# kuwt/model_matching

Measured on AMD Instinct MI355X. Metric: candidate poses verified/sec, higher is better.
Workload: dtype f32; 1 GPU; Cm: synthetic 20000-pt scene vs 5000-pt model, 65536 candidate transforms per step per GPU, eps=5mm; scene_points=20000, model_points=5000

## Files before the change

model_matching_amd/csrc/lcp.hip:

```cpp
#include <stdlib.h>
#include <string.h>

#include <cstring>


#include <algorithm>
#include <utility>

#include "kdtree.h"
#include "prims.h"
#include "stocs_ctx.h"

namespace stocs {

struct LcpArgs {
    const float4* mpos;
    const float4* mnrm;
    const int32_t* mperm;
    int M;
    const int32_t* top;
    const uint4* cells;
    const uint4* flat;
    const float4* list;
    const float4* snrmw;
// ... 165 lines not shown
    __shared__ unsigned long long part[WPB];
    const int lane = threadIdx.x & 63;
    const int sub = lane & 7, grp = lane >> 3;
    const int w = threadIdx.x >> 6;
    const int cand = SPLIT ? lcp_candidate(a, n, 0, 1) : lcp_candidate(a, n, w, WPB);
    if (cand < 0) return;
    const int first = SPLIT ? 64 * w : 0, stride = SPLIT ? 64 * WPB : 64;
    const float4* __restrict__ snrmw = lcp_weights_of(a, cand);
    const float* T = T16 + (size_t)cand * 16;
    const float t0 = T[0], t1 = T[1], t2 = T[2], t4 = T[4], t5 = T[5], t6 = T[6], t8 = T[8], t9 = T[9], t10 = T[10],
                t12 = T[12], t13 = T[13], t14 = T[14];
    unsigned long long acc = 0ull;
    for (int base = first; base < a.M; base += stride) {
        const int i = base + lane;
        float qx = 0.f, qy = 0.f, qz = 0.f, qcd = 0.f;
        uint32_t off = 0, cnt = 0;
        if (i < a.M) {
            const float4 p = a.mpos[i];
            qx = ((t0 * p.x + t4 * p.y) + t8 * p.z) + t12;
            qy = ((t1 * p.x + t5 * p.y) + t9 * p.z) + t13;
            qz = ((t2 * p.x + t6 * p.y) + t10 * p.z) + t14;
            const float ux = (qx - a.ox) * a.inv_h, uy = (qy - a.oy) * a.inv_h, uz = (qz - a.oz) * a.inv_h;
            const float fx = floorf(ux), fy = floorf(uy), fz = floorf(uz);
            if (fx >= 0.0f && fy >= 0.0f && fz >= 0.0f && fx < (float)a.nx && fy < (float)a.ny && fz < (float)a.nz) {
                const int cx = (int)fx, cy = (int)fy, cz = (int)fz;
                const int brick = STOCS_ABLATE(a, 1) ? -1 : a.top[((cz >> 3) * a.nby + (cy >> 3)) * a.nbx + (cx >> 3)];
                if (brick >= 0) {
                    uint4 cw = make_uint4(0u, 0u, 0u, 0u);
                    if (!STOCS_ABLATE(a, 128)) cw = a.cells[(size_t)brick * 512 + (((cz & 7) << 6) | ((cy & 7) << 3) | (cx & 7))];
                    const int sb = ((int)((uz - fz) * 4.0f) << 4) | ((int)((uy - fy) * 4.0f) << 2) | (int)((ux - fx) * 4.0f);
                    const uint32_t mw = a.has_nearest ? 0xFFFFFFFFu : (sb < 32 ? cw.z : cw.w);
                    off = cw.x; cnt = ((mw >> (sb & 31)) & 1u) ? cw.y : 0u;
                    if (STOCS_ABLATE(a, 2)) cnt = cw.x == 0xFFFFFFF1u ? 1u : 0u;
                    const float ex = qx - (a.ox + ((float)cx + 0.5f) * a.h), ey = qy - (a.oy + ((float)cy + 0.5f) * a.h),
                                ez = qz - (a.oz + ((float)cz + 0.5f) * a.h);
                    qcd = sqrtf(ex * ex + (ey * ey + ez * ez));
                }
            }
        }
        const bool hit = cnt != 0;
        const unsigned long long mask = __ballot(hit);
        int best = -1;
        if (mask) {
            const int nh = __popcll(mask);
            if (hit) {
                const int rank = __popcll(mask & ((1ull << lane) - 1ull));
                hl[w][rank] = (uint32_t)lane;
                qt[w][lane] = make_float4(qx, qy, qz, __int_as_float((int)off));
                qn[w][lane] = cnt;
                qd[w][lane] = qcd;
            }
            __builtin_amdgcn_wave_barrier();
            for (int s = 0; s < nh; s += 8) {
                const int slot = s + grp;
                const bool gact = slot < nh;
                const uint32_t L = gact ? hl[w][slot] : 0u;
                const float4 qq = qt[w][L];
                const uint32_t c = gact ? qn[w][L] : 0u;
                const float4* lp = a.list + (uint32_t)__float_as_int(qq.w) + sub;
                float gd = a.sq_eps;
                int gi = -1;
                const float qcg = qd[w][L];
                const uint32_t chunk0 = (uint32_t)__float_as_int(qq.w) >> 3;
                uint32_t nchunks = (c + 7u) >> 3;
                float gb = a.sq_eps;
                if (STOCS_ABLATE(a, 4)) nchunks = min(nchunks, (uint32_t)UNR);
                for (uint32_t j = 0; __any(j < nchunks); j += UNR) {
                    if (j < nchunks && j > 0 && (STOCS_ABLATE(a, 256) ? 0.0f : a.chunk_r[chunk0 + j]) - qcg > sqrtf(gb) + a.bound_margin) nchunks = 0;
                    float4 e[UNR];
#pragma unroll
                    for (int u = 0; u < UNR; ++u) {
                        e[u] = make_float4(1e30f, 1e30f, 1e30f, __int_as_float(-1));
                        if (j + u < nchunks) e[u] = lp[(j + u) << 3];
                    }
#pragma unroll
                    for (int u = 0; u < UNR; ++u) {
                        const float dx = qq.x - e[u].x, dy = qq.y - e[u].y, dz = qq.z - e[u].z;
                        const float d = dx * dx + (dy * dy + dz * dz);
                        const int ei = __float_as_int(e[u].w);
                        if (d < gd || (d == gd && ei > gi)) { gd = d; gi = ei; }
                    }
                    gb = fminf(gd, dpp_f32<DPP_QUAD_XOR1>(gd));
                    gb = fminf(gb, dpp_f32<DPP_QUAD_XOR2>(gb));
                    gb = fminf(gb, dpp_f32<DPP_HALF_MIRROR>(gb));
                }
                float dm = fminf(gd, dpp_f32<DPP_QUAD_XOR1>(gd));
                dm = fminf(dm, dpp_f32<DPP_QUAD_XOR2>(dm));
                dm = fminf(dm, dpp_f32<DPP_HALF_MIRROR>(dm));
                int im = (gd == dm) ? gi : -1;
                im = max(im, dpp_i32<DPP_QUAD_XOR1>(im));
                im = max(im, dpp_i32<DPP_QUAD_XOR2>(im));
                im = max(im, dpp_i32<DPP_HALF_MIRROR>(im));
                if (gact && sub == 0) { rd[w][L] = dm; ri[w][L] = im; }
            }
            __builtin_amdgcn_wave_barrier();
            if (hit) best = ri[w][lane];
            __builtin_amdgcn_wave_barrier();
        }
        bool counted = false;
        if (best >= 0 && STOCS_ABLATE(a, 8)) lcp_add(acc, 0.5f);
        else if (best >= 0) {
            const float4 nm = a.mnrm[i];
            const float nx = t0 * nm.x + (t4 * nm.y + t8 * nm.z);
            const float ny = t1 * nm.x + (t5 * nm.y + t9 * nm.z);
            const float nz = t2 * nm.x + (t6 * nm.y + t10 * nm.z);
            const float4 sn = snrmw[best];
            const float d = sn.x * nx + (sn.y * ny + sn.z * nz);
            counted = (d >= a.dot_lo) && (d <= 1.0f);
            if (counted) lcp_add(acc, sn.w);
        }
        if (DETAIL && i < a.M) {
            const int orig = a.mperm[i];
            hit_out[(size_t)cand * a.M + orig] = best;
            cnt_out[(size_t)cand * a.M + orig] = counted ? 1 : 0;
        }
    }
    acc = lcp_wave_sum(acc);
    if (SPLIT) {
        if (lane == 0) part[w] = acc;
        __syncthreads();
        if (threadIdx.x == 0) {
            unsigned long long total = 0;
#pragma unroll
            for (int k = 0; k < WPB; ++k) total += part[k];
            lcp_store(a, out, cand, total);
        }
    } else if (lane == 0) lcp_store(a, out, cand, acc);
}

__device__ __forceinline__ float lcp_linear_norm_bound(float t0, float t1, float t2, float t4, float t5, float t6, float t8, float t9, float t10) {
    const float g00 = t0 * t0 + (t1 * t1 + t2 * t2), g11 = t4 * t4 + (t5 * t5 + t6 * t6), g22 = t8 * t8 + (t9 * t9 + t10 * t10);
    const float g01 = fabsf(t0 * t4 + (t1 * t5 + t2 * t6)), g02 = fabsf(t0 * t8 + (t1 * t9 + t2 * t10)), g12 = fabsf(t4 * t8 + (t5 * t9 + t6 * t10));
    const float rho = fmaxf(g00 + (g01 + g02), fmaxf(g11 + (g01 + g12), g22 + (g02 + g12)));
    return sqrtf(rho) * 1.00001f;
}
__device__ __forceinline__ bool lcp_patch_dead(const LcpArgs& a, const float4 sp, float sn, float t0, float t1, float t2, float t4, float t5, float t6,
                                               float t8, float t9, float t10, float t12, float t13, float t14) {
    const float cx = ((t0 * sp.x + t4 * sp.y) + t8 * sp.z) + t12;
    const float cy = ((t1 * sp.x + t5 * sp.y) + t9 * sp.z) + t13;
    const float cz = ((t2 * sp.x + t6 * sp.y) + t10 * sp.z) + t14;
    const float mag = fabsf(cx) + (fabsf(cy) + fabsf(cz));
    if (!(mag < 1.0e18f)) return false;
    const float need = (sn * sp.w + a.eps * 1.002f) + (4.0e-6f + 4.0e-6f * mag);
    const float ux = (cx - a.gox) * a.inv_g, uy = (cy - a.goy) * a.inv_g, uz = (cz - a.goz) * a.inv_g;
    const float fx = floorf(ux), fy = floorf(uy), fz = floorf(uz);
    if (fx >= 1.0f && fy >= 1.0f && fz >= 1.0f && fx < (float)(a.gnx - 1) && fy < (float)(a.gny - 1) && fz < (float)(a.gnz - 1)) {
        const float v = a.dist[((uint32_t)(int)fz * (uint32_t)a.gny + (uint32_t)(int)fy) * (uint32_t)a.gnx + (uint32_t)(int)fx];
        const float ex = cx - (a.gox + (fx + 0.5f) * a.g), ey = cy - (a.goy + (fy + 0.5f) * a.g), ez = cz - (a.goz + (fz + 0.5f) * a.g);
        return v - sqrtf(ex * ex + (ey * ey + ez * ez)) > need;
    }
    return a.cap > need;
}

constexpr bool lcp_queue_form_legal(bool detail, bool dense, bool split, bool flat, bool near, int cu) {
    return (cu == 16 || cu == 64) && (detail ? (!split && !flat && !(dense && near)) : (!dense || (split && !flat && !near)));
}

template <bool DETAIL, bool DENSE, bool SPLIT, bool FLAT, bool NEAR, int CU>
__global__ __launch_bounds__(64 * lcp_waves_per_block(DETAIL, SPLIT), 8) void lcp_coopq_kernel(LcpArgs a, const float* __restrict__ T16, float* __restrict__ out,
                                                        int n, int32_t* __restrict__ hit_out, uint8_t* __restrict__ cnt_out) {
    static_assert(lcp_queue_form_legal(DETAIL, DENSE, SPLIT, FLAT, NEAR, CU), "not one of the forms in the table above");
    constexpr int WPB = lcp_waves_per_block(DETAIL, SPLIT);
    constexpr bool IDX = !DENSE;
    constexpr bool EARLY = DENSE;
    constexpr int GL = 4, EPL = 8 / GL, NG = 64 / GL;
    constexpr int FIRST = DENSE ? 1 : 2, E0 = EPL * FIRST;
    constexpr bool NOSENT = !DENSE;
    constexpr int UNR = 1;
    constexpr int PIPE = 1;
    static_assert(!EARLY || (FIRST == 1 && !NOSENT), "early exit decides line by line");
    __shared__ float4 qt[WPB][128];
    __shared__ float qcd[EARLY ? WPB : 1][EARLY ? 128 : 1];
    __shared__ uint32_t qn[WPB][128];
    __shared__ uint32_t qs[WPB][128];
    __shared__ int ri[WPB][128];
    __shared__ uint8_t ord[WPB][64];
    __shared__ unsigned long long part[WPB];
    const int lane = threadIdx.x & 63;
    const int w = threadIdx.x >> 6;
    const int cand = SPLIT ? lcp_candidate(a, n, 0, 1) : lcp_candidate(a, n, w, WPB);
    if (cand < 0) return;
    const float4* __restrict__ snrmw = lcp_weights_of(a, cand);
    const float* T = T16 + (size_t)cand * 16;
    const float t0 = T[0], t1 = T[1], t2 = T[2], t4 = T[4], t5 = T[5], t6 = T[6], t8 = T[8], t9 = T[9], t10 = T[10],
                t12 = T[12], t13 = T[13], t14 = T[14];
    unsigned long long acc = 0ull;
    int head = 0, tail = 0;

    auto process = [&](int nq) {
        {
            uint32_t cls = 4;
            if (lane < nq) {
                const uint32_t nch = (qn[w][(head + lane) & 127] + 7u) >> 3;
                cls = nch <= (uint32_t)FIRST ? 1u : (nch <= (uint32_t)(FIRST + UNR) ? 2u : 3u);
            }
            const unsigned long long below = (1ull << lane) - 1ull;
            const unsigned long long m1 = __ballot(cls == 1u), m2 = __ballot(cls == 2u), m3 = __ballot(cls == 3u);
            const int n1 = __popcll(m1), n2 = __popcll(m2);
            const int pos = cls == 1u ? __popcll(m1 & below) : (cls == 2u ? n1 + __popcll(m2 & below) : n1 + n2 + __popcll(m3 & below));
            if (lane < nq) ord[w][pos] = (uint8_t)lane;
            __builtin_amdgcn_wave_barrier();
        }
        for (int s0 = 0; s0 < nq; s0 += NG * PIPE) {
            const int sub = lane & (GL - 1), grp = lane / GL;
            float4 e0[PIPE][E0];
            bool wide[PIPE];
            int idxs[PIPE];
            uint32_t cs[PIPE];
#pragma unroll
            for (int u = 0; u < PIPE; ++u) {
                const int slot = s0 + NG * u + grp;
                const bool gact = slot < nq;
                idxs[u] = (head + (int)ord[w][gact ? slot : 0]) & 127;
                cs[u] = gact ? qn[w][idxs[u]] : 0u;
                wide[u] = true;
                if (!NOSENT) {
#pragma unroll
                    for (int e = 0; e < E0; ++e) e0[u][e] = make_float4(1e30f, 1e30f, 1e30f, __int_as_float(-1));
                }
                if (STOCS_ABLATE(a, 4)) {
                    if (cs[u]) { const float4 qq0 = qt[w][idxs[u]]; e0[u][0] = make_float4(qq0.x, qq0.y, qq0.z, __int_as_float(0)); }
                    cs[u] = cs[u] ? 1u : 0u;
                }
                else if (NOSENT) {
                    const float4* l0 = a.list + (cs[u] ? (uint32_t)__float_as_int(qt[w][idxs[u]].w) : 0u) + sub;
                    const uint32_t last = cs[u] ? ((cs[u] - 1u) & ~7u) : 0u;
#pragma unroll
                    for (int e = 0; e < EPL; ++e) e0[u][e] = l0[GL * e];
                    wide[u] = FIRST > 1 && __any(cs[u] > 8u);
                    if (wide[u]) {
#pragma unroll
                        for (int e = EPL; e < E0; ++e) e0[u][e] = l0[min((uint32_t)(8 * (e / EPL)), last) + GL * (e % EPL)];
                    }
                }
                else if (cs[u]) {
                    const float4* l0 = a.list + (uint32_t)__float_as_int(qt[w][idxs[u]].w) + sub;
#pragma unroll
                    for (int e = 0; e < E0; ++e) e0[u][e] = l0[GL * e];
                }
            }
#pragma unroll
            for (int u = 0; u < PIPE; ++u) {
                const float4 qq = qt[w][idxs[u]];
                const uint32_t c = cs[u];
                const float4* lp = a.list + (uint32_t)__float_as_int(qq.w) + sub;
                const uint32_t last_line = c ? ((c - 1u) & ~7u) : 0u;
                float gd = a.sq_eps;
                int gi = -1;
#pragma unroll
                for (int e = 0; e < EPL; ++e) {
                    const float dx = qq.x - e0[u][e].x, dy = qq.y - e0[u][e].y, dz = qq.z - e0[u][e].z;
                    const float d = dx * dx + (dy * dy + dz * dz);
                    take_if_better<IDX>(d, __float_as_int(e0[u][e].w), gd, gi);
                }
                if (FIRST > 1 && wide[u]) {
#pragma unroll
                    for (int e = EPL; e < E0; ++e) {
                        const float dx = qq.x - e0[u][e].x, dy = qq.y - e0[u][e].y, dz = qq.z - e0[u][e].z;
                        const float d = dx * dx + (dy * dy + dz * dz);
                        take_if_better<IDX>(d, __float_as_int(e0[u][e].w), gd, gi);
                    }
                }
                if (EARLY) {
                    const float qcg = qcd[w][idxs[u]];
                    const uint32_t chunk0 = (uint32_t)__float_as_int(qq.w) >> 3;
                    uint32_t cc = c;
                    for (uint32_t k = 8; __any(k < cc); k += 8 * UNR) {
                        if (k < cc && a.chunk_r[chunk0 + (k >> 3)] - qcg > sqrtf(group_min_nonneg<GL>(gd)) + a.bound_margin) cc = 0;
                        float4 e[EPL];
                        if (k < cc) {
#pragma unroll
                            for (int x = 0; x < EPL; ++x) e[x] = lp[k + GL * x];
                        } else {
#pragma unroll
                            for (int x = 0; x < EPL; ++x) e[x] = make_float4(1e30f, 1e30f, 1e30f, __int_as_float(-1));
                        }
#pragma unroll
                        for (int x = 0; x < EPL; ++x) {
                            const float dx = qq.x - e[x].x, dy = qq.y - e[x].y, dz = qq.z - e[x].z;
                            const float d = dx * dx + (dy * dy + dz * dz);
                            take_if_better<IDX>(d, __float_as_int(e[x].w), gd, gi);
                        }
                    }
                } else {
                    for (uint32_t k = 8 * FIRST; __any(k < c); k += 8 * UNR) {
                        const uint32_t kk = min(k, last_line);
                        float4 e[EPL];
#pragma unroll
                        for (int x = 0; x < EPL; ++x) e[x] = lp[kk + GL * x];
#pragma unroll
                        for (int x = 0; x < EPL; ++x) {
                            const float dx = qq.x - e[x].x, dy = qq.y - e[x].y, dz = qq.z - e[x].z;
                            const float d = dx * dx + (dy * dy + dz * dz);
                            take_if_better<IDX>(d, __float_as_int(e[x].w), gd, gi);
                        }
                    }
                }
                const float dm = group_min_nonneg<GL>(gd);
                int im = (gd == dm) ? gi : -1;
                im = max(im, dpp_i32<DPP_QUAD_XOR1>(im));
                im = max(im, dpp_i32<DPP_QUAD_XOR2>(im));
                if (c && sub == 0) ri[w][idxs[u]] = im;
            }
        }
        __builtin_amdgcn_wave_barrier();
        if (lane < nq) {
            const int idx = (head + lane) & 127;
            const int best = ri[w][idx];
            const uint32_t slot_i = qs[w][idx];
            bool counted = false;
            if (best >= 0 && STOCS_ABLATE(a, 8)) { lcp_add(acc, 0.5f); }
            else if (best >= 0) {
                const float4 nm = STOCS_ABLATE(a, 16) ? make_float4(0.f, 0.f, 1.f, 0.f) : a.mnrm[slot_i];
                const float nx = t0 * nm.x + (t4 * nm.y + t8 * nm.z);
                const float ny = t1 * nm.x + (t5 * nm.y + t9 * nm.z);
                const float nz = t2 * nm.x + (t6 * nm.y + t10 * nm.z);
                const float4 sn = STOCS_ABLATE(a, 32) ? make_float4(nx, ny, nz, 0.5f) : snrmw[best];
                const float d = sn.x * nx + (sn.y * ny + sn.z * nz);
                counted = (d >= a.dot_lo) && (d <= 1.0f);
                if (counted) lcp_add(acc, sn.w);
            }
            if (DETAIL) {
                const int orig = a.mperm[slot_i];
                hit_out[(size_t)cand * a.M + orig] = best;
                cnt_out[(size_t)cand * a.M + orig] = counted ? 1 : 0;
            }
        }
        __builtin_amdgcn_wave_barrier();
    };

    auto step = [&](const int i, const float4 p) {
        float qx = 0.f, qy = 0.f, qz = 0.f, qcentre = 0.f, nearest = 0.f;
        uint32_t off = 0, cnt = 0;
        if (!DETAIL || i < a.M) {
            qx = ((t0 * p.x + t4 * p.y) + t8 * p.z) + t12;
            qy = ((t1 * p.x + t5 * p.y) + t9 * p.z) + t13;
            qz = ((t2 * p.x + t6 * p.y) + t10 * p.z) + t14;
            const int c4x = __float2int_rd((qx - a.ox) * a.inv_h4), c4y = __float2int_rd((qy - a.oy) * a.inv_h4),
                      c4z = __float2int_rd((qz - a.oz) * a.inv_h4);
            const int cx = c4x >> 2, cy = c4y >> 2, cz = c4z >> 2;
            if ((unsigned)cx < (unsigned)a.nx && (unsigned)cy < (unsigned)a.ny && (unsigned)cz < (unsigned)a.nz) {
                const int sb = ((c4z & 3) << 4) | ((c4y & 3) << 2) | (c4x & 3);
                if (FLAT) {
                    uint4 cw = make_uint4(0u, 0u, 0u, 0u);
                    if (!STOCS_ABLATE(a, 1))
                        cw = a.flat[(uint32_t)((cz * a.ny + cy) * a.nx + cx)];
                    const uint32_t mw = sb < 32 ? cw.z : cw.w;
                    off = cw.x; cnt = ((mw >> (sb & 31)) & 1u) ? cw.y : 0u;
                    if (STOCS_ABLATE(a, 2)) cnt = cw.x == 0xFFFFFFF1u ? 1u : 0u;
                } else {
                    const int brick = a.top[((cz >> 3) * a.nby + (cy >> 3)) * a.nbx + (cx >> 3)];
                    if (brick >= 0) {
                        const uint4 cw = a.cells[(uint32_t)brick * 512u + (uint32_t)(((cz & 7) << 6) | ((cy & 7) << 3) | (cx & 7))];
                        if ((EARLY || NEAR) && a.has_nearest) { off = cw.x; cnt = cw.y; nearest = __uint_as_float(cw.z); }
                        else { const uint32_t mw = a.has_nearest ? 0xFFFFFFFFu : (sb < 32 ? cw.z : cw.w); off = cw.x; cnt = ((mw >> (sb & 31)) & 1u) ? cw.y : 0u; }
                    }
                }
            }
            if ((EARLY || (NEAR && a.has_nearest)) && cnt) {
                const float ex = qx - (a.ox + ((float)cx + 0.5f) * a.h), ey = qy - (a.oy + ((float)cy + 0.5f) * a.h), ez = qz - (a.oz + ((float)cz + 0.5f) * a.h);
                qcentre = sqrtf(ex * ex + (ey * ey + ez * ez));
                if (a.has_nearest && nearest - qcentre > a.eps + a.bound_margin) cnt = 0;
            }
            if (DETAIL && cnt == 0) {
                const int orig = a.mperm[i];
                hit_out[(size_t)cand * a.M + orig] = -1;
                cnt_out[(size_t)cand * a.M + orig] = 0;
            }
        }
        const bool hit = cnt != 0;
        const unsigned long long mask = __ballot(hit);
        if (mask) {
            if (hit) {
                const int rank = __popcll(mask & ((1ull << lane) - 1ull));
                const int sl = (tail + rank) & 127;
                qt[w][sl] = make_float4(qx, qy, qz, __int_as_float((int)off));
                qn[w][sl] = cnt;
                qs[w][sl] = (uint32_t)i;
                if (EARLY) qcd[w][sl] = qcentre;
            }
            tail += __popcll(mask);
            __builtin_amdgcn_wave_barrier();
            if (tail - head >= 64) {
                process(64);
                head += 64;
            }
        }
    };
    if (CU == 16) {
    __shared__ uint16_t live_q[WPB][128];
    const int nsteps = (a.M + 63) >> 6;
    const int wfirst = SPLIT ? w : 0, nw = SPLIT ? WPB : 1;
    const int nsub = __builtin_amdgcn_readfirstlane(4 * ((nsteps - wfirst + nw - 1) / nw));
    const float snorm = a.patch ? lcp_linear_norm_bound(t0, t1, t2, t4, t5, t6, t8, t9, t10) : 0.0f;
    int qh = 0, qtl = 0;
    for (int s0 = 0;; s0 += 64) {
        {
            const int kl = s0 + lane, q = 4 * (wfirst + (kl >> 2) * nw) + (kl & 3);
            const bool in = kl < nsub && (q << 4) < a.M;
            bool live = in;
            if (a.patch && live && !STOCS_ABLATE(a, 64))
                live = !lcp_patch_dead(a, a.sub[q], snorm, t0, t1, t2, t4, t5, t6, t8, t9, t10, t12, t13, t14);
            const unsigned long long mask = __ballot(live);
            if (live) live_q[w][(qtl + __popcll(mask & ((1ull << lane) - 1ull))) & 127] = (uint16_t)q;
            qtl += __popcll(mask);
            if (DETAIL && a.patch) {
                unsigned long long dead = __ballot(in && !live);
                while (dead) {
                    const int j = __builtin_ctzll(dead);
                    dead &= dead - 1ull;
                    const int id = ((4 * (wfirst + ((s0 + j) >> 2) * nw) + ((s0 + j) & 3)) << 4) + lane;
                    if (lane < 16 && id < a.M) {
                        const int orig = a.mperm[id];
                        hit_out[(size_t)cand * a.M + orig] = -1;
                        cnt_out[(size_t)cand * a.M + orig] = 0;
                    }
                }
            }
            __builtin_amdgcn_wave_barrier();
        }
        const bool last = s0 + 64 >= nsub;
        const int g = lane >> 4;
        auto slot = [&](int t) { return g < t ? ((int)live_q[w][(qh + g) & 127] << 4) + (lane & 15) : (nsteps << 6) + lane; };
        int t = min(qtl - qh, 4);
        if (t == 4 || (last && t > 0)) {
            int i = slot(t);
            float4 p_next = a.mpos[i];
            for (;;) {
                const int ic = i;
                const float4 p = p_next;
                qh += t;
                t = min(qtl - qh, 4);
                const bool more = t == 4 || (last && t > 0);
                i = more ? slot(t) : ic;
                p_next = a.mpos[i];
                step(ic, p);
                if (!more) break;
            }
        }
        if (last) break;
    }
    } else {
    const int nsteps = (a.M + 63) >> 6;
    const int wfirst = SPLIT ? w : 0, nw = SPLIT ? WPB : 1;
    const int nk = (nsteps - wfirst + nw - 1) / nw;
    const float snorm = a.patch ? lcp_linear_norm_bound(t0, t1, t2, t4, t5, t6, t8, t9, t10) : 0.0f;
    for (int k0 = 0; k0 < nk; k0 += 64) {
        const int kk = k0 + lane;
        bool live = kk < nk;
        if (a.patch && live && !STOCS_ABLATE(a, 64))
            live = !lcp_patch_dead(a, a.patch[wfirst + kk * nw], snorm, t0, t1, t2, t4, t5, t6, t8, t9, t10, t12, t13, t14);
        unsigned long long todo = __ballot(live);
        if (DETAIL && a.patch) {
            unsigned long long dead = __ballot(kk < nk && !live);
            while (dead) {
                const int j = __builtin_ctzll(dead);
                dead &= dead - 1ull;
                const int i = ((wfirst + (k0 + j) * nw) << 6) + lane;
                if (i < a.M) {
                    const int orig = a.mperm[i];
                    hit_out[(size_t)cand * a.M + orig] = -1;
                    cnt_out[(size_t)cand * a.M + orig] = 0;
                }
            }
        }
        if (!todo) continue;
        int j = __builtin_ctzll(todo);
        float4 p_next = a.mpos[((wfirst + (k0 + j) * nw) << 6) + lane];
        for (;;) {
            const int i = ((wfirst + (k0 + j) * nw) << 6) + lane;
            const float4 p = p_next;
            todo &= todo - 1ull;
            j = todo ? __builtin_ctzll(todo) : j;
            p_next = a.mpos[((wfirst + (k0 + j) * nw) << 6) + lane];
            step(i, p);
            if (!todo) break;
        }
    }
    }
    if (tail - head > 0) process(tail - head);
    acc = lcp_wave_sum(acc);
    if (SPLIT) {
        if (lane == 0) part[w] = acc;
        __syncthreads();
        if (threadIdx.x == 0) {
            unsigned long long total = 0;
#pragma unroll
            for (int k = 0; k < WPB; ++k) total += part[k];
            lcp_store(a, out, cand, total);
        }
    } else if (lane == 0) lcp_store(a, out, cand, acc);
}

template <bool DETAIL>
__global__ __launch_bounds__(256) void lcp_exact_kernel(LcpArgs a, const float* __restrict__ T16, float* __restrict__ out, int n,
                                                        int32_t* __restrict__ hit_out, uint8_t* __restrict__ cnt_out,
                                                        const KdNodeP* __restrict__ kd_nodes, const float4* __restrict__ kd_pts,
                                                        unsigned long long* __restrict__ ties) {
    const int lane = threadIdx.x & 63;
    const int cand = lcp_candidate(a, n, threadIdx.x >> 6);
    if (cand < 0) return;
    const float* T = T16 + (size_t)cand * 16;
    const float4* __restrict__ snrmw = lcp_weights_of(a, cand);
    const float t0 = T[0], t1 = T[1], t2 = T[2], t4 = T[4], t5 = T[5], t6 = T[6], t8 = T[8], t9 = T[9], t10 = T[10],
                t12 = T[12], t13 = T[13], t14 = T[14];
    unsigned long long acc = 0ull, n_flag = 0ull, n_changed = 0ull;
    for (int i = lane; i < a.M; i += 64) {
        const float4 p = a.mpos[i];
        const float qx = ((t0 * p.x + t4 * p.y) + t8 * p.z) + t12;
        const float qy = ((t1 * p.x + t5 * p.y) + t9 * p.z) + t13;
        const float qz = ((t2 * p.x + t6 * p.y) + t10 * p.z) + t14;
        const float fx = floorf((qx - a.ox) * a.inv_h);
        const float fy = floorf((qy - a.oy) * a.inv_h);
        const float fz = floorf((qz - a.oz) * a.inv_h);
        int best = -1;
        bool tie = false;
        float bd = a.sq_eps;
        if (fx >= 0.0f && fy >= 0.0f && fz >= 0.0f && fx < (float)a.nx && fy < (float)a.ny && fz < (float)a.nz) {
            const int cx = (int)fx, cy = (int)fy, cz = (int)fz;
            const int brick = a.top[((cz >> 3) * a.nby + (cy >> 3)) * a.nbx + (cx >> 3)];
            if (brick >= 0) {
                const uint4 cw = a.cells[(size_t)brick * 512 + (((cz & 7) << 6) | ((cy & 7) << 3) | (cx & 7))];
                for (uint32_t k = 0; k < cw.y; ++k) {
                    const float4 s = a.list[cw.x + k];
                    const float dx = qx - s.x, dy = qy - s.y, dz = qz - s.z;
                    const float d = dx * dx + (dy * dy + dz * dz);
                    const int ei = __float_as_int(s.w);
                    if (d < bd) { bd = d; best = ei; tie = false; }
                    else if (d == bd) { if (best >= 0) { tie = true; best = max(best, ei); } else best = ei; }
                }
            }
        }
        if (tie || (best >= 0 && bd == a.sq_eps)) {
            const int kb = kd_query_closest(kd_nodes, kd_pts, qx, qy, qz, a.sq_eps);
            n_flag++;
            if (kb != best) n_changed++;
            best = kb;
        }
        bool counted = false;
        if (best >= 0) {
            const float4 nm = a.mnrm[i];
            const float nx = t0 * nm.x + (t4 * nm.y + t8 * nm.z);
            const float ny = t1 * nm.x + (t5 * nm.y + t9 * nm.z);
            const float nz = t2 * nm.x + (t6 * nm.y + t10 * nm.z);
            const float4 sn = snrmw[best];
            const float d = sn.x * nx + (sn.y * ny + sn.z * nz);
            counted = (d >= a.dot_lo) && (d <= 1.0f);
            if (counted) lcp_add(acc, sn.w);
        }
        if (DETAIL) {
            const int orig = a.mperm[i];
            hit_out[(size_t)cand * a.M + orig] = best;
            cnt_out[(size_t)cand * a.M + orig] = counted ? 1 : 0;
        }
    }
    acc = lcp_wave_sum(acc);
    n_flag = lcp_wave_sum(n_flag);
    n_changed = lcp_wave_sum(n_changed);
    if (lane == 0) {
        lcp_store(a, out, cand, acc);
        if (n_flag) atomicAdd(&ties[0], n_flag);
        if (n_changed) atomicAdd(&ties[1], n_changed);
    }
}

__global__ __launch_bounds__(256) void best_kernel(const float* __restrict__ lcp, int n, uint32_t id_offset, unsigned long long* __restrict__ best) {
    unsigned long long k = 0;
    for (int i = blockIdx.x * blockDim.x + threadIdx.x; i < n; i += gridDim.x * blockDim.x) {
        const float s = lcp[i];
        if (s > 0.0f) {
            const unsigned long long key = ((unsigned long long)__float_as_uint(s) << 32) | (unsigned long long)(0xFFFFFFFFu - (id_offset + (uint32_t)i));
            k = key > k ? key : k;
        }
    }
    for (int off = 32; off > 0; off >>= 1) {
        const unsigned long long o = __shfl_xor(k, off, 64);
        k = o > k ? o : k;
    }
    if ((threadIdx.x & 63) == 0 && k) atomicMax(best, k);
}

__global__ __launch_bounds__(1024) void best_single_kernel(const float* __restrict__ lcp, int n, uint32_t id_offset, unsigned long long* __restrict__ best) {
    __shared__ unsigned long long sh[16];
    unsigned long long k = 0;
    for (int i = threadIdx.x; i < n; i += 1024) {
        const float s = lcp[i];
        if (s > 0.0f) {
            const unsigned long long key = ((unsigned long long)__float_as_uint(s) << 32) | (unsigned long long)(0xFFFFFFFFu - (id_offset + (uint32_t)i));
            k = key > k ? key : k;
        }
    }
    for (int off = 32; off > 0; off >>= 1) {
        const unsigned long long o = __shfl_xor(k, off, 64);
        k = o > k ? o : k;
    }
    if ((threadIdx.x & 63) == 0) sh[threadIdx.x >> 6] = k;
    __syncthreads();
    if (threadIdx.x == 0) {
        for (int w = 1; w < 16; ++w) k = sh[w] > k ? sh[w] : k;
        *best = k;
    }
}

__device__ __forceinline__ uint32_t spread10(uint32_t x) {
    x &= 0x3ff; x = (x | (x << 16)) & 0x30000ff; x = (x | (x << 8)) & 0x300f00f; x = (x | (x << 4)) & 0x30c30c3; x = (x | (x << 2)) & 0x9249249;
    return x;
}
__global__ __launch_bounds__(256) void order_keys_kernel(const float* __restrict__ T16, int n, float ox, float oy, float oz, float sx, float sy, float sz,
                                                         uint32_t* __restrict__ keys, int32_t* __restrict__ vals, unsigned long long* __restrict__ best) {
    const int i = blockIdx.x * blockDim.x + threadIdx.x;
    if (i == 0 && best) *best = 0ull;
    if (i >= n) return;
    const float* T = T16 + (size_t)i * 16;
    const float qx = fminf(fmaxf((T[12] - ox) * sx, 0.0f), 255.0f), qy = fminf(fmaxf((T[13] - oy) * sy, 0.0f), 255.0f),
                qz = fminf(fmaxf((T[14] - oz) * sz, 0.0f), 255.0f);
    keys[i] = (spread10((uint32_t)qz) << 2) | (spread10((uint32_t)qy) << 1) | spread10((uint32_t)qx);
    vals[i] = i;
}

enum LcpKernel { LCP_PLAIN, LCP_STEP, LCP_QUEUE, LCP_EXACT };
struct LcpForm {
    LcpKernel kernel;
    bool detail;
    bool dense;
    bool split;
    bool flat, near;
    int cu;
};

static bool lcp_variant_selectable(int v) { return v == 99 || v == 0 || v == 24 || v == 31 || v == 39; }

static LcpForm choose_lcp_form(const stocs_ctx* c, const LcpArgs& a, bool detail) {
    LcpForm f = {LCP_QUEUE, detail, false, false, false, false, 64};
    if (c->exact_ties) { f.kernel = LCP_EXACT; return f; }
    f.dense = c->grid.d_chunk_r != NULL;
    const int variant = c->lcp_variant >= 0 ? c->lcp_variant : 99;
    if (variant == 0) f.kernel = (detail && f.dense) ? LCP_STEP : LCP_PLAIN;
    else if (variant == 31 && f.dense) f.kernel = LCP_STEP;
    const bool split = c->lcp_split && a.M >= 512;
    if (f.kernel == LCP_STEP) f.split = !detail && split;
    if (f.kernel == LCP_QUEUE) {
        f.split = !detail && (f.dense || split);
        f.flat = !detail && !f.dense && c->lcp_flat && a.flat;
        f.near = !f.dense && a.has_nearest;
        f.cu = (a.patch && c->lcp_cull_unit == 16) ? 16 : 64;
    }
    return f;
}

typedef void (*LcpScanFn)(LcpArgs, const float*, float*, int, int32_t*, uint8_t*);

template <int I>
static LcpScanFn lcp_queue_fn() {
    constexpr bool DETAIL = (I & 1) != 0, DENSE = (I & 2) != 0, SPLIT = (I & 4) != 0, FLAT = (I & 8) != 0, NEAR = (I & 16) != 0;
    constexpr int CU = (I & 32) ? 16 : 64;
    if constexpr (lcp_queue_form_legal(DETAIL, DENSE, SPLIT, FLAT, NEAR, CU)) return lcp_coopq_kernel<DETAIL, DENSE, SPLIT, FLAT, NEAR, CU>;
    else return NULL;
}
template <int... I>
static LcpScanFn lcp_queue_fn(const LcpForm& f, std::integer_sequence<int, I...>) {
    static const LcpScanFn table[] = {lcp_queue_fn<I>()...};
    return table[(f.detail ? 1 : 0) | (f.dense ? 2 : 0) | (f.split ? 4 : 0) | (f.flat ? 8 : 0) | (f.near ? 16 : 0) | (f.cu == 16 ? 32 : 0)];
}

static int launch_lcp_form(stocs_ctx* c, const LcpForm& f, const LcpArgs& a, const float* d_T16, int n, float* d_lcp, int32_t* d_hit, uint8_t* d_counted) {
    const bool cooperative = f.kernel == LCP_STEP || f.kernel == LCP_QUEUE;
    const bool one_wave = cooperative && !f.detail && !f.split;
    const dim3 grid((unsigned)(f.split || one_wave ? n : (n + 3) / 4)), block(one_wave ? 64 : 256);
    if (f.kernel == LCP_EXACT) {
        if (f.detail) hipLaunchKernelGGL(lcp_exact_kernel<true>, grid, block, 0, c->stream, a, d_T16, d_lcp, n, d_hit, d_counted, c->d_kd_nodes, c->d_kd_pts, c->d_ties);
        else hipLaunchKernelGGL(lcp_exact_kernel<false>, grid, block, 0, c->stream, a, d_T16, d_lcp, n, d_hit, d_counted, c->d_kd_nodes, c->d_kd_pts, c->d_ties);
    } else {
        LcpScanFn fn = NULL;
        if (f.kernel == LCP_QUEUE) fn = lcp_queue_fn(f, std::make_integer_sequence<int, 64>());
        else if (f.kernel == LCP_STEP) fn = f.detail ? lcp_coop_kernel<true, false> : (f.split ? lcp_coop_kernel<false, true> : lcp_coop_kernel<false, false>);
        else if (!f.detail) fn = f.dense ? lcp_kernel<false, false> : lcp_kernel<false, true>;
        else if (!f.dense) fn = lcp_kernel<true, true>;
        if (!fn) { set_error("launch_lcp: no kernel for this form (kernel %d, detail %d, dense %d, split %d, flat %d, near %d, cu %d)", (int)f.kernel, (int)f.detail, (int)f.dense, (int)f.split, (int)f.flat, (int)f.near, f.cu); return STOCS_ERR_STATE; }
        hipLaunchKernelGGL(fn, grid, block, 0, c->stream, a, d_T16, d_lcp, n, d_hit, d_counted);
    }
    STOCS_HIP_CHECK(hipGetLastError());
    return STOCS_OK;
}

int launch_lcp(stocs_ctx* c, const float* d_T16, int n, float* d_lcp, int32_t* d_hit, uint8_t* d_counted, unsigned long long* d_best8, uint32_t id_offset) {
    if (n <= 0) { if (d_best8) STOCS_HIP_CHECK(hipMemsetAsync(d_best8, 0, 8, c->stream)); return STOCS_OK; }
    bool best_zeroed = false;
    LcpArgs a;
    a.best = d_best8; a.id_offset = id_offset;
#ifdef STOCS_TOOLS_BUILD
    a.ablate = getenv("STOCS_LCP_ABLATE") ? atoi(getenv("STOCS_LCP_ABLATE")) : 0;
#endif
    a.mpos = c->d_mpos_s; a.mnrm = c->d_mnrm_s; a.mperm = c->d_mperm; a.M = c->nM;
    a.top = c->grid.d_top; a.cells = c->grid.d_cells; a.flat = c->grid.d_flat; a.list = c->grid.d_list; a.snrmw = c->snrmw_override ? c->snrmw_override : c->d_snrmw;
    a.cand_trial = c->lcp_cand_trial; a.snrmw_stride = c->lcp_cand_trial ? c->snrmw_stride : 0;
    a.ox = c->grid.ox; a.oy = c->grid.oy; a.oz = c->grid.oz; a.inv_h = c->grid.inv_h; a.inv_h4 = c->grid.inv_h * 4.0f; a.h = c->grid.h; a.chunk_r = c->grid.d_chunk_r;
    a.nx = c->grid.nx; a.ny = c->grid.ny; a.nz = c->grid.nz; a.nbx = c->grid.nbx; a.nby = c->grid.nby;
    a.sq_eps = c->prm.distance_threshold * c->prm.distance_threshold;
    a.dot_lo = c->thr.lcp_dot_lo;
    a.eps = c->prm.distance_threshold;
    a.has_nearest = c->grid.has_nearest ? 1 : 0;
    {
        double mag = 0.0;
        for (int k = 0; k < 3; ++k) mag = std::max(mag, std::max(fabs(c->grid.bb_mn[k]), fabs(c->grid.bb_mx[k])));
        a.bound_margin = (float)(4.0e-4 * (double)c->prm.distance_threshold + 4.0e-6 * mag);
    }
    a.patch = NULL; a.sub = NULL; a.dist = NULL;
    a.gox = a.goy = a.goz = 0.f; a.g = a.inv_g = a.cap = 0.f; a.gnx = a.gny = a.gnz = 0;
    c->scene_scored++;
    c->scene_work += (double)n * (double)c->nM;
    if (c->exact_ties) {
        int rc = ensure_kdtree(c);
        if (rc) return rc;
        if (!c->ties_started) { STOCS_HIP_CHECK(hipMemsetAsync(c->d_ties, 0, 16, c->stream)); c->ties_started = true; }
        a.order = NULL; a.xcd_blocks = 0;
        if (d_best8 && !(d_best8 == c->d_best && c->best_is_zero)) STOCS_HIP_CHECK(hipMemsetAsync(d_best8, 0, 8, c->stream));
        if (d_best8 == c->d_best) c->best_is_zero = false;
        return launch_lcp_form(c, choose_lcp_form(c, a, d_hit != NULL), a, d_T16, n, d_lcp, d_hit, d_counted);
    }
    if (c->lcp_cull && c->grid.d_dist && c->d_mpatch && (c->grid.dist_ready || c->lcp_cull >= 2 || c->scene_work >= c->lcp_cull_after)) {
        int rc = fill_cull_field(c);
        if (rc) return rc;
        if (c->cull_pending) { STOCS_HIP_CHECK(hipStreamWaitEvent(c->stream, c->ev_cull, 0)); c->cull_pending = false; }
        a.patch = c->d_mpatch; a.sub = c->d_msub; a.dist = c->grid.d_dist;
        a.gox = c->grid.cg_ox; a.goy = c->grid.cg_oy; a.goz = c->grid.cg_oz; a.g = c->grid.cg_g; a.inv_g = c->grid.cg_inv_g; a.cap = c->grid.cg_cap;
        a.gnx = c->grid.cg_nx; a.gny = c->grid.cg_ny; a.gnz = c->grid.cg_nz;
    }
    a.order = NULL; a.xcd_blocks = 0;
    const bool lists_spill = (double)c->grid.n_entries * 16.0 >= 12.0e6;
    if (!d_hit && n >= 1024 && (double)n * (double)c->nM >= 1.5e8 && c->lcp_order && (lists_spill || c->lcp_order >= 2)) {
        const size_t kb = (((size_t)n * 4 + 255) / 256) * 256;
        size_t tb = 0;
        STOCS_HIP_CHECK(sort_pairs(NULL, tb, (const uint32_t*)NULL, (uint32_t*)NULL, (const uint32_t*)NULL, (uint32_t*)NULL, (size_t)n, 0, 24, c->stream));
        const size_t need = 4 * kb + tb;
        if (c->order_bytes < need) {
            if (c->d_order) { STOCS_HIP_CHECK(hipStreamSynchronize(c->stream)); (void)hipFree(c->d_order); c->d_order = NULL; c->order_bytes = 0; }
            STOCS_HIP_CHECK(dev_malloc(&c->d_order, need + need / 4));
            c->order_bytes = need + need / 4;
        }
        char* p = (char*)c->d_order;
        uint32_t* keys = (uint32_t*)p; uint32_t* keys_s = (uint32_t*)(p + kb);
        int32_t* vals = (int32_t*)(p + 2 * kb); int32_t* order = (int32_t*)(p + 3 * kb);
        void* tmp = p + 4 * kb;
        const float sx = 256.0f / ((float)c->grid.nx * c->grid.h), sy = 256.0f / ((float)c->grid.ny * c->grid.h), sz = 256.0f / ((float)c->grid.nz * c->grid.h);
        hipLaunchKernelGGL(order_keys_kernel, dim3((unsigned)((n + 255) / 256)), dim3(256), 0, c->stream, d_T16, n, c->grid.ox, c->grid.oy, c->grid.oz, sx, sy, sz,
                           keys, vals, d_best8);
        best_zeroed = true;
        STOCS_HIP_CHECK(sort_pairs(tmp, tb, keys, keys_s, (const uint32_t*)vals, (uint32_t*)order, (size_t)n, 0, 24, c->stream));
        a.order = order;
        const bool lists_huge = (double)c->grid.n_entries * 16.0 >= 512.0e6;
        a.xcd_blocks = c->lcp_order >= 2 ? (c->lcp_order == 2 ? 1 : c->lcp_order) : (lists_huge ? 128 : 0);
    }
    if (d_best8 && d_best8 == c->d_best && c->best_is_zero) best_zeroed = true;
    if (d_best8 == c->d_best) c->best_is_zero = false;
    if (d_best8 && !best_zeroed) STOCS_HIP_CHECK(hipMemsetAsync(d_best8, 0, 8, c->stream));
    return launch_lcp_form(c, choose_lcp_form(c, a, d_hit != NULL), a, d_T16, n, d_lcp, d_hit, d_counted);
}

static int enqueue_best(stocs_ctx* c, const float* d_lcp, int n, uint32_t id_offset, unsigned long long* d_key8) {
    if (n <= (1 << 18)) {
        hipLaunchKernelGGL(best_single_kernel, dim3(1), dim3(1024), 0, c->stream, d_lcp, n, id_offset, d_key8);
    } else {
        STOCS_HIP_CHECK(hipMemsetAsync(d_key8, 0, 8, c->stream));
        const int blocks = std::min((n + 255) / 256, 1024);
        hipLaunchKernelGGL(best_kernel, dim3(blocks), dim3(256), 0, c->stream, d_lcp, n, id_offset, d_key8);
    }
    STOCS_HIP_CHECK(hipGetLastError());
    return STOCS_OK;
}

static int read_best_key(stocs_ctx* c, uint64_t* key) {
    int rc = ensure_pinned(c, PIN_VAR);
    if (rc) return rc;
    uint64_t* key_pin = (uint64_t*)((char*)c->h_pin + PIN_BEST);
    STOCS_HIP_CHECK(hipMemcpyAsync(key_pin, c->d_best, 8, hipMemcpyDeviceToHost, c->stream));
    STOCS_HIP_CHECK(hipStreamSynchronize(c->stream));
    *key = *key_pin;
    return STOCS_OK;
}

}

using namespace stocs;

extern "C" {

int stocs_score_transforms_device(stocs_ctx* c, const void* d_T16, int n, void* d_lcp) {
    if (!c || n < 0 || (n && (!d_T16 || !d_lcp))) return STOCS_ERR_INVALID;
    DeviceGuard dev_guard(c->device);
    begin_scoring_call(c);
    return launch_lcp(c, (const float*)d_T16, n, (float*)d_lcp, NULL, NULL, NULL, 0);
}

int stocs_score_transforms(stocs_ctx* c, const float* T_host, int n, float* lcp_host) {
    if (!c || n < 0 || (n && (!T_host || !lcp_host))) return STOCS_ERR_INVALID;
    DeviceGuard dev_guard(c->device);
    begin_scoring_call(c);
    if (n == 0) return STOCS_OK;
    const size_t tb = (size_t)n * 64, lb = (size_t)n * 4;
    int rc = ensure_scratch(c, tb + lb + 256);
    if (rc) return rc;
    float* dT = (float*)c->d_scratch;
    float* dL = (float*)((char*)c->d_scratch + ((tb + 255) / 256) * 256);
    STOCS_HIP_CHECK(hipMemcpyAsync(dT, T_host, tb, hipMemcpyHostToDevice, c->stream));
    rc = launch_lcp(c, dT, n, dL, NULL, NULL, NULL, 0);
    if (rc) return rc;
    STOCS_HIP_CHECK(hipMemcpyAsync(lcp_host, dL, lb, hipMemcpyDeviceToHost, c->stream));
    STOCS_HIP_CHECK(hipStreamSynchronize(c->stream));
    return STOCS_OK;
}

int stocs_lcp_detail(stocs_ctx* c, const float* T_host, int32_t* hit, uint8_t* counted) {
    if (!c || !T_host || !hit || !counted) return STOCS_ERR_INVALID;
    DeviceGuard dev_guard(c->device);
    begin_scoring_call(c);
    const size_t M = (size_t)c->nM;
    int rc = ensure_scratch(c, 256 + 256 + M * 4 + 256 + M);
    if (rc) return rc;
    char* base = (char*)c->d_scratch;
    float* dT = (float*)base;
    float* dL = (float*)(base + 256);
    int32_t* dH = (int32_t*)(base + 512);
    uint8_t* dC = (uint8_t*)(base + 512 + ((M * 4 + 255) / 256) * 256);
    STOCS_HIP_CHECK(hipMemcpyAsync(dT, T_host, 64, hipMemcpyHostToDevice, c->stream));
    rc = launch_lcp(c, dT, 1, dL, dH, dC, NULL, 0);
    if (rc) return rc;
    STOCS_HIP_CHECK(hipMemcpyAsync(hit, dH, M * 4, hipMemcpyDeviceToHost, c->stream));
    STOCS_HIP_CHECK(hipMemcpyAsync(counted, dC, M, hipMemcpyDeviceToHost, c->stream));
    STOCS_HIP_CHECK(hipStreamSynchronize(c->stream));
    return STOCS_OK;
}
// ... 147 lines not shown
```

Before: 71.63 million poses/s.

## Share one block-wide live patch list across waves in split cu16 LCP kernel

Adds a SHARED variant of the cooperative queue kernel for split forms with 16-point cull units and a model of at most 8192 points. All waves cull model sub-patches together and append the survivors to a single block-wide list in shared memory through an LDS atomic. Each wave then takes an even share of the surviving steps instead of keeping its own ring over a fixed stride of patches. This aims to even out load across waves when culling leaves them uneven work. The cost is two block barriers, and the dispatch table doubles to 128 template instances.

```diff
diff --git a/model_matching_amd/csrc/lcp.hip b/model_matching_amd/csrc/lcp.hip
--- a/model_matching_amd/csrc/lcp.hip
+++ b/model_matching_amd/csrc/lcp.hip
@@ -341,14 +341,16 @@
     return a.cap > need;
 }
 
-constexpr bool lcp_queue_form_legal(bool detail, bool dense, bool split, bool flat, bool near, int cu) {
-    return (cu == 16 || cu == 64) && (detail ? (!split && !flat && !(dense && near)) : (!dense || (split && !flat && !near)));
-}
-
-template <bool DETAIL, bool DENSE, bool SPLIT, bool FLAT, bool NEAR, int CU>
+constexpr int LCP_SHARED_LIVE = 512;
+
+constexpr bool lcp_queue_form_legal(bool detail, bool dense, bool split, bool flat, bool near, int cu, bool shared) {
+    return (cu == 16 || cu == 64) && (!shared || (split && cu == 16)) && (detail ? (!split && !flat && !(dense && near)) : (!dense || (split && !flat && !near)));
+}
+
+template <bool DETAIL, bool DENSE, bool SPLIT, bool FLAT, bool NEAR, int CU, bool SHARED>
 __global__ __launch_bounds__(64 * lcp_waves_per_block(DETAIL, SPLIT), 8) void lcp_coopq_kernel(LcpArgs a, const float* __restrict__ T16, float* __restrict__ out,
                                                         int n, int32_t* __restrict__ hit_out, uint8_t* __restrict__ cnt_out) {
-    static_assert(lcp_queue_form_legal(DETAIL, DENSE, SPLIT, FLAT, NEAR, CU), "not one of the forms in the table above");
+    static_assert(lcp_queue_form_legal(DETAIL, DENSE, SPLIT, FLAT, NEAR, CU, SHARED), "not one of the forms in the table above");
     constexpr int WPB = lcp_waves_per_block(DETAIL, SPLIT);
     constexpr bool IDX = !DENSE;
     constexpr bool EARLY = DENSE;
@@ -579,6 +581,51 @@
     if (CU == 16) {
     __shared__ uint16_t live_q[WPB][128];
     const int nsteps = (a.M + 63) >> 6;
+    if (SHARED) {
+    __shared__ int live_n;
+    uint16_t* const live_all = &live_q[0][0];
+    static_assert(!SHARED || WPB * 128 == LCP_SHARED_LIVE, "the shared list is the memory of the per-wave rings");
+    if (threadIdx.x == 0) live_n = 0;
+    const int nsubs = (a.M + 15) >> 4;
+    const float snorm = a.patch ? lcp_linear_norm_bound(t0, t1, t2, t4, t5, t6, t8, t9, t10) : 0.0f;
+    unsigned long long lm[2];
+#pragma unroll
+    for (int j = 0; j < 2; ++j) {
+        const int q = ((w + 4 * j) << 6) + lane;
+        bool live = q < nsubs;
+        if (a.patch && live && !STOCS_ABLATE(a, 64))
+            live = !lcp_patch_dead(a, a.sub[q], snorm, t0, t1, t2, t4, t5, t6, t8, t9, t10, t12, t13, t14);
+        lm[j] = __ballot(live);
+    }
+    __syncthreads();
+#pragma unroll
+    for (int j = 0; j < 2; ++j) {
+        if (lm[j]) {
+            int base = 0;
+            if (lane == 0) base = atomicAdd(&live_n, __popcll(lm[j]));
+            base = __builtin_amdgcn_readfirstlane(base);
+            if ((lm[j] >> lane) & 1ull)
+                live_all[base + __popcll(lm[j] & ((1ull << lane) - 1ull))] = (uint16_t)(((w + 4 * j) << 6) + lane);
+        }
+    }
+    __syncthreads();
+    const int nlive = __builtin_amdgcn_readfirstlane(live_n);
+    const int nst = (nlive + 3) >> 2;
+    const int mine = __builtin_amdgcn_readfirstlane((nst + 3 - w) >> 2);
+    const int e0 = 4 * w + (lane >> 4);
+    auto slot = [&](int k) { const int e = e0 + 16 * k; return e < nlive ? ((int)live_all[e] << 4) + (lane & 15) : (nsteps << 6) + lane; };
+    if (mine > 0) {
+        int i = slot(0);
+        float4 p_next = a.mpos[i];
+        for (int k = 0; k < mine; ++k) {
+            const int ic = i;
+            const float4 p = p_next;
+            i = k + 1 < mine ? slot(k + 1) : ic;
+            p_next = a.mpos[i];
+            step(ic, p);
+        }
+    }
+    } else {
     const int wfirst = SPLIT ? w : 0, nw = SPLIT ? WPB : 1;
     const int nsub = __builtin_amdgcn_readfirstlane(4 * ((nsteps - wfirst + nw - 1) / nw));
     const float snorm = a.patch ? lcp_linear_norm_bound(t0, t1, t2, t4, t5, t6, t8, t9, t10) : 0.0f;
@@ -628,6 +675,7 @@
             }
         }
         if (last) break;
+    }
     }
     } else {
     const int nsteps = (a.M + 63) >> 6;
@@ -815,12 +863,13 @@
     bool split;
     bool flat, near;
     int cu;
+    bool shared;
 };
 
 static bool lcp_variant_selectable(int v) { return v == 99 || v == 0 || v == 24 || v == 31 || v == 39; }
 
 static LcpForm choose_lcp_form(const stocs_ctx* c, const LcpArgs& a, bool detail) {
-    LcpForm f = {LCP_QUEUE, detail, false, false, false, false, 64};
+    LcpForm f = {LCP_QUEUE, detail, false, false, false, false, 64, false};
     if (c->exact_ties) { f.kernel = LCP_EXACT; return f; }
     f.dense = c->grid.d_chunk_r != NULL;
     const int variant = c->lcp_variant >= 0 ? c->lcp_variant : 99;
@@ -833,6 +882,7 @@
         f.flat = !detail && !f.dense && c->lcp_flat && a.flat;
         f.near = !f.dense && a.has_nearest;
         f.cu = (a.patch && c->lcp_cull_unit == 16) ? 16 : 64;
+        f.shared = f.split && f.cu == 16 && a.M <= 16 * LCP_SHARED_LIVE;
     }
     return f;
 }
@@ -843,13 +893,14 @@
 static LcpScanFn lcp_queue_fn() {
     constexpr bool DETAIL = (I & 1) != 0, DENSE = (I & 2) != 0, SPLIT = (I & 4) != 0, FLAT = (I & 8) != 0, NEAR = (I & 16) != 0;
     constexpr int CU = (I & 32) ? 16 : 64;
-    if constexpr (lcp_queue_form_legal(DETAIL, DENSE, SPLIT, FLAT, NEAR, CU)) return lcp_coopq_kernel<DETAIL, DENSE, SPLIT, FLAT, NEAR, CU>;
+    constexpr bool SHARED = (I & 64) != 0;
+    if constexpr (lcp_queue_form_legal(DETAIL, DENSE, SPLIT, FLAT, NEAR, CU, SHARED)) return lcp_coopq_kernel<DETAIL, DENSE, SPLIT, FLAT, NEAR, CU, SHARED>;
     else return NULL;
 }
 template <int... I>
 static LcpScanFn lcp_queue_fn(const LcpForm& f, std::integer_sequence<int, I...>) {
     static const LcpScanFn table[] = {lcp_queue_fn<I>()...};
-    return table[(f.detail ? 1 : 0) | (f.dense ? 2 : 0) | (f.split ? 4 : 0) | (f.flat ? 8 : 0) | (f.near ? 16 : 0) | (f.cu == 16 ? 32 : 0)];
+    return table[(f.detail ? 1 : 0) | (f.dense ? 2 : 0) | (f.split ? 4 : 0) | (f.flat ? 8 : 0) | (f.near ? 16 : 0) | (f.cu == 16 ? 32 : 0) | (f.shared ? 64 : 0)];
 }
 
 static int launch_lcp_form(stocs_ctx* c, const LcpForm& f, const LcpArgs& a, const float* d_T16, int n, float* d_lcp, int32_t* d_hit, uint8_t* d_counted) {
@@ -861,11 +912,11 @@
         else hipLaunchKernelGGL(lcp_exact_kernel<false>, grid, block, 0, c->stream, a, d_T16, d_lcp, n, d_hit, d_counted, c->d_kd_nodes, c->d_kd_pts, c->d_ties);
     } else {
         LcpScanFn fn = NULL;
-        if (f.kernel == LCP_QUEUE) fn = lcp_queue_fn(f, std::make_integer_sequence<int, 64>());
+        if (f.kernel == LCP_QUEUE) fn = lcp_queue_fn(f, std::make_integer_sequence<int, 128>());
         else if (f.kernel == LCP_STEP) fn = f.detail ? lcp_coop_kernel<true, false> : (f.split ? lcp_coop_kernel<false, true> : lcp_coop_kernel<false, false>);
         else if (!f.detail) fn = f.dense ? lcp_kernel<false, false> : lcp_kernel<false, true>;
         else if (!f.dense) fn = lcp_kernel<true, true>;
-        if (!fn) { set_error("launch_lcp: no kernel for this form (kernel %d, detail %d, dense %d, split %d, flat %d, near %d, cu %d)", (int)f.kernel, (int)f.detail, (int)f.dense, (int)f.split, (int)f.flat, (int)f.near, f.cu); return STOCS_ERR_STATE; }
+        if (!fn) { set_error("launch_lcp: no kernel for this form (kernel %d, detail %d, dense %d, split %d, flat %d, near %d, cu %d, shared %d)", (int)f.kernel, (int)f.detail, (int)f.dense, (int)f.split, (int)f.flat, (int)f.near, f.cu, (int)f.shared); return STOCS_ERR_STATE; }
         hipLaunchKernelGGL(fn, grid, block, 0, c->stream, a, d_T16, d_lcp, n, d_hit, d_counted);
     }
     STOCS_HIP_CHECK(hipGetLastError());
```

Result: faster. 73.32 million poses/s, median of 6 (+2.4%).
